# 0xC0000054/pdn-jpegxl

Hardware: AMD Instinct MI355X
Metric: megapixels/sec decode (4K lossy VarDCT) (higher is better)
Workload: dtype f32

## Files before the change

pdn_jpegxl_amd/csrc/dev_util.h:

```cpp
#pragma once
#include <stdint.h>
#include <hip/hip_fp16.h>

namespace jxlhip {

__host__ __device__ __forceinline__ int ReflectIndex(int v, int n) {
  while (v < 0 || v >= n) v = v < 0 ? -v - 1 : 2 * n - 1 - v;
  return v;
}

__host__ __device__ __forceinline__ size_t OrientedIndex(int o, int x, int y, int w, int h) {
  int ox, oy;
  switch (o) {
    case 2: ox = w - 1 - x; oy = y; break;
    case 3: ox = w - 1 - x; oy = h - 1 - y; break;
    case 4: ox = x; oy = h - 1 - y; break;
    case 5: ox = y; oy = x; break;
    case 6: ox = h - 1 - y; oy = x; break;
    case 7: ox = h - 1 - y; oy = w - 1 - x; break;
    case 8: ox = y; oy = w - 1 - x; break;
    default: ox = x; oy = y; break;
  }
  return (size_t)oy * (size_t)(o >= 5 ? h : w) + (size_t)ox;
}

__host__ __device__ __forceinline__ uint32_t NnzBucketCtx(uint32_t nzl) {
  const uint32_t b = (nzl >= 2) + (nzl >= 3) + (nzl >= 5) + (nzl >= 9) + (nzl >= 13) + (nzl >= 21) + (nzl >= 33);
  return (uint32_t)(0xCEB4987B5D3E1F00ull >> (8 * b)) & 0xFFu;
}

__host__ __device__ __forceinline__ uint32_t HfPosCtx(uint32_t ks) {
  const uint32_t a = ks - 1, b = 7 + (ks >> 1), c = 15 + (ks >> 2);
  const uint32_t bc = b < c ? b : c;
  return a < bc ? a : bc;
}

__host__ __device__ __forceinline__ uint32_t HfNnzPredict(uint32_t bx, uint32_t by, uint32_t above, uint32_t left) {
  return bx == 0 ? (by == 0 ? 32u : above) : (by == 0 ? left : (above + left + 1) >> 1);
}
__host__ __device__ __forceinline__ uint32_t HfNnzCountBucket(uint32_t predicted) {
  const uint32_t p = predicted >= 64 ? 64 : predicted;
  return p < 8 ? p : 4 + p / 2;
}

__device__ __forceinline__ uint32_t IntToOutSample(int32_t v, int bits, int out_bits) {
  const int32_t maxv = (int32_t)((1u << bits) - 1);
  if (bits == out_bits) return (uint32_t)min(maxv, max(0, v));
  float f = (float)v * (1.0f / (float)maxv);
  f *= out_bits == 16 ? 65535.0f : 255.0f;
  const float top = out_bits == 16 ? 65535.0f : 255.0f;
  if (!(f > 0.f)) return 0;
  if (f >= top) return (uint32_t)top;
  return (uint32_t)(f + 0.5f);
}

__device__ __forceinline__ float BitsToFloatSample(int32_t v, int bits) {
  if (bits == 32) return __int_as_float(v);
  return __half2float(__ushort_as_half((unsigned short)(v & 0xFFFF)));
}
__device__ __forceinline__ uint32_t FloatToOutBits(float f, int out_bits, int out_float) {
  if (out_float) return out_bits == 32 ? (uint32_t)__float_as_int(f) : (uint32_t)__half_as_ushort(__float2half_rn(f));
  const float top = out_bits == 16 ? 65535.0f : 255.0f;
  f *= top;
  if (!(f > 0.f)) return 0;
  if (f >= top) return (uint32_t)top;
  return (uint32_t)(f + 0.5f);
}
__device__ __forceinline__ uint32_t SampleToOutBits(int32_t v, int bits, int exp_bits, int out_bits, int out_float) {
  if (!out_float && !exp_bits) return IntToOutSample(v, bits, out_bits);
  const float f = exp_bits ? BitsToFloatSample(v, bits) : (float)v * (1.0f / (float)((1u << bits) - 1));
  return FloatToOutBits(f, out_bits, out_float);
}
__device__ __forceinline__ void StoreOutSample(uint8_t* base, size_t index, uint32_t raw, int out_bits) {
  if (out_bits == 8) base[index] = (uint8_t)raw;
  else if (out_bits == 16) ((uint16_t*)base)[index] = (uint16_t)raw;
  else ((uint32_t*)base)[index] = raw;
}

}
```

pdn_jpegxl_amd/csrc/entropy_kernels.hip:

```cpp
#include <hip/hip_runtime.h>
#include <cstdlib>
#include <type_traits>
#include "dev_types.h"
#include "dev_util.h"
#include "kernels.h"
#include "lds_layout.h"
#include "modular_rules.h"

namespace jxlhip {

namespace {

__device__ const uint8_t d_order_bucket[kNumStrategies] = {0, 1, 1, 1, 2, 3, 4, 4, 5, 5, 6, 6, 1, 1, 1, 1, 1, 1, 7, 8, 8, 9, 10, 10, 11, 12, 12};
__device__ const uint8_t d_log2cx[kNumStrategies] = {0, 0, 0, 0, 1, 2, 0, 1, 0, 2, 1, 2, 0, 0, 0, 0, 0, 0, 3, 2, 3, 4, 3, 4, 5, 4, 5};
__device__ const uint8_t d_log2cy[kNumStrategies] = {0, 0, 0, 0, 1, 2, 1, 0, 2, 0, 2, 1, 0, 0, 0, 0, 0, 0, 3, 3, 2, 4, 4, 3, 5, 5, 4};
__device__ const uint8_t d_nnz_ctx[64] = {0,   0,   31,  62,  62,  93,  93,  93,  93,  123, 123, 123, 123, 152, 152, 152, 152, 152, 152, 152, 152, 180,
                                          180, 180, 180, 180, 180, 180, 180, 180, 180, 180, 180, 206, 206, 206, 206, 206, 206, 206, 206, 206, 206, 206,
                                          206, 206, 206, 206, 206, 206, 206, 206, 206, 206, 206, 206, 206, 206, 206, 206, 206, 206, 206, 206};

__device__ __forceinline__ int CeilLog2D(uint32_t x) { return x <= 1 ? 0 : 32 - __clz(x - 1); }
#ifndef JXLHIP_PRIO_SERIAL
#define JXLHIP_PRIO_SERIAL 0
#endif
#if JXLHIP_PRIO_SERIAL
// ... 1090 lines not shown
    for (uint32_t i = i0; i < i1; i++) {
      const int es = s_info[i];
      s_pre[i] = base;
      base += (es >= 0 && es < kNumStrategies) ? 1u << d_log2cx[es] : 1u;
    }
    if (err & kErrBlockLayout) atomicOr(&s_flag, 1u);
  }
  __threadfence_block();
  __syncthreads();
  uint32_t num = 0;
  bool layout_bad = false;
  if (!s_flag) {
    const int words = (bw + 31) >> 5;
    for (int y = 0; y < bh; y++) {
      uint32_t pre[9];
      pre[0] = 0;
#pragma unroll
      for (int wi = 0; wi < 8; wi++) {
        uint32_t fr = 0;
        if (wi < words) {
          fr = ~s_cov[y * 8 + wi];
          const int lim = min(32, bw - wi * 32);
          if (lim < 32) fr &= (1u << lim) - 1;
        }
        pre[wi + 1] = pre[wi] + (uint32_t)__popc(fr);
      }
      const uint32_t nfree = pre[8];
      bool inrow = false, bad = false;
      if (nfree) {
        const uint32_t j = num + (uint32_t)tid;
        uint32_t off = 0;
        if (j < count) { off = s_pre[j] - s_pre[num]; inrow = off < nfree; }
        if (inrow) {
          const int es = s_info[j];
          const int lcx = d_log2cx[es], lcy = d_log2cy[es], cx = 1 << lcx, cy = 1 << lcy;
          int wi = 0;
          uint32_t before = 0;
#pragma unroll
          for (int k = 1; k < 8; k++) { const bool past = pre[k] <= off; wi += past ? 1 : 0; before = past ? pre[k] : before; }
          uint32_t word = ~s_cov[y * 8 + wi];
          const int lim = min(32, bw - wi * 32);
          if (lim < 32) word &= (1u << lim) - 1;
          uint32_t rem = off - before;
          int xb = 0;
#pragma unroll
          for (int sft = 16; sft; sft >>= 1) {
            const uint32_t c = (uint32_t)__popc((word >> xb) & ((1u << sft) - 1));
            if (rem >= c) { rem -= c; xb += sft; }
          }
          const int x = wi * 32 + xb;
          const uint32_t mask = (cx == 32 ? 0xFFFFFFFFu : ((1u << cx) - 1)) << xb;
          if (off + (uint32_t)cx > nfree || x + cx > bw || y + cy > bh || xb + cx > 32 || (y & 31) + cy > 32 || (word & mask) != mask) {
            bad = true;
          } else {
            for (int iy = 1; iy < cy; iy++)
              if (atomicOr(&s_cov[(y + iy) * 8 + wi], mask) & mask) bad = true;
            s_pos[j] = x | y << 8;
          }
        }
      }
      const int n_row = __syncthreads_count(inrow);
      if (nfree && s_pre[num + (uint32_t)n_row] - s_pre[num] != nfree) bad = true;
      if (__syncthreads_or(bad)) { layout_bad = true; break; }
      num += (uint32_t)n_row;
    }
  }
  __threadfence_block();
  __syncthreads();
  if (s_flag || layout_bad || num != count) err |= kErrBlockLayout;
  if (tid == 0) s_count = (err & kErrBlockLayout) ? 0u : num;
  __syncthreads();
  const uint32_t placed = s_count;
  for (uint32_t i = tid; i < placed; i += 256) {
    const int x = s_pos[i] & 0xFF, y = s_pos[i] >> 8;
    const int s = s_info[i], q = 1 + s_info[count + i];
    const int lcx = d_log2cx[s], lcy = d_log2cy[s], cx = 1 << lcx, cy = 1 << lcy;
    const size_t cell = (size_t)(by0 + y) * im.w8 + bx0 + x;
    for (int iy = 0; iy < cy; iy++)
      for (int ix = 0; ix < cx; ix++) {
        const size_t cc = cell + (size_t)iy * im.w8 + ix;
        im.cellinfo[cc] = (uint32_t)s | ix << 8 | iy << 13 | lcx << 18 | lcy << 21 | 1u << 31;
        im.rawq[cc] = (uint16_t)q;
      }
  }
  if (err) SetError(im, err, 2, g);
}

__global__ __launch_bounds__(64) void hf_blocklist_kernel(const DevImage* __restrict__ imgs) {
  const DevImage& im = imgs[blockIdx.y];
  const int g = blockIdx.x;
  if (g >= im.ng || im.is_modular) return;
  const int lane = threadIdx.x;
  const int gx = g % im.xg, gy = g / im.xg;
  const int bx0 = gx * kGroupBlocks, by0 = gy * kGroupBlocks;
  const int bw = min(kGroupBlocks, im.w8 - bx0), bh = min(kGroupBlocks, im.h8 - by0);
  uint32_t* list = im.blk_list + (size_t)g * 1024;
  const int n_qf = im.n_qf;
  uint32_t total = 0;
  for (int it = 0; it < 16; it++) {
    const int idx = it * 64 + lane;
    const int bx = idx & 31, by = idx >> 5;
    bool first = false;
    uint32_t info = 0;
    if (bx < bw && by < bh) {
      info = im.cellinfo[(size_t)(by0 + by) * im.w8 + bx0 + bx];
      first = (info & 0x8003FF00u) == 0x80000000u;
    }
    const uint64_t m = __ballot(first);
    if (first) {
      const uint32_t pos = total + (uint32_t)__popcll(m & (((uint64_t)1 << lane) - 1));
      const uint32_t s = info & 0xFF, lcx = (info >> 18) & 7, lcy = (info >> 21) & 7;
      const uint32_t ord = d_order_bucket[s];
      const uint32_t rq = im.rawq[(size_t)(by0 + by) * im.w8 + bx0 + bx];
      uint32_t qf_idx = 0;
      for (int i = 0; i < n_qf; i++) qf_idx += rq > im.qf_thr[i];
      uint32_t lf_idx = 0;
      if (im.num_lf_ctx > 1) {
        const size_t cell = (size_t)(by0 + by) * im.w8 + bx0 + bx;
        uint32_t ix = 0, iy = 0, ib = 0;
        for (int i = 0; i < im.n_lf_thr[0]; i++) ix += im.lfq[0][cell] > im.lf_thr[0][i];
        for (int i = 0; i < im.n_lf_thr[1]; i++) iy += im.lfq[1][cell] > im.lf_thr[1][i];
        for (int i = 0; i < im.n_lf_thr[2]; i++) ib += im.lfq[2][cell] > im.lf_thr[2][i];
        lf_idx = (ix * (uint32_t)(im.n_lf_thr[2] + 1) + ib) * (uint32_t)(im.n_lf_thr[1] + 1) + iy;
      }
      uint32_t ctxs = 0;
      for (int ci = 0; ci < 3; ci++) {
        const int c = ci == 0 ? 1 : (ci == 1 ? 0 : 2);
        const uint32_t cprime = c < 2 ? (c ^ 1) : 2;
        ctxs |= ((uint32_t)im.block_ctx_map[((cprime * kNumOrders + ord) * (n_qf + 1) + qf_idx) * im.num_lf_ctx + lf_idx] & 31u) << (5 * ci);
      }
      list[pos] = (uint32_t)bx | (uint32_t)by << 5 | lcx << 10 | lcy << 13 | ctxs << 16;
    }
    total += (uint32_t)__popcll(m);
  }
  if (lane == 0) im.blk_count[g] = total;
}

namespace {

constexpr int kHfTop = kHfRingWords / 2;
constexpr int kHfQ = kHfQueueDepth;
constexpr uint32_t kHfDqMask = 2u * kHfQ - 1;
typedef LaneBitsT<kHfRingWords, kHfRingWords / 4> HfBits;
typedef ScalarBitsT<kHfRingWords> HfScalarBits;

struct HfProfile {
#ifdef JXLHIP_PROFILE_HF
  uint64_t start = clock64(), scalar = 0, period = 0, tokens = 0, entries = 0, periods = 0, general = 0, general_n = 0;
  __device__ __forceinline__ uint64_t Now() const { return clock64(); }
  __device__ __forceinline__ void Period(uint64_t t0) { periods++; period += clock64() - t0; }
  __device__ __forceinline__ void ScalarRun(uint64_t t0, uint32_t n) { entries++; scalar += clock64() - t0; tokens += n; }
  __device__ __forceinline__ uint64_t GeneralBegin() { general_n++; return clock64(); }
  __device__ __forceinline__ void GeneralEnd(uint64_t t0) { general += clock64() - t0; }
  __device__ __forceinline__ void Print(int g, uint32_t nblk, int per_wave) const {
    if (per_wave == 1)
      printf("[hfprof] g %d total %llu scalar-loop %llu (%llu entries, %llu tokens) period %llu (%llu periods) blocks %u general %llu (%llu iterations)\n", g,
             (unsigned long long)(clock64() - start), (unsigned long long)scalar, (unsigned long long)entries, (unsigned long long)tokens,
             (unsigned long long)period, (unsigned long long)periods, nblk, (unsigned long long)general, (unsigned long long)general_n);
  }
#else
  __device__ __forceinline__ uint64_t Now() const { return 0; }
  __device__ __forceinline__ void Period(uint64_t) {}
  __device__ __forceinline__ void ScalarRun(uint64_t, uint32_t) {}
  __device__ __forceinline__ uint64_t GeneralBegin() { return 0; }
  __device__ __forceinline__ void GeneralEnd(uint64_t) {}
  __device__ __forceinline__ void Print(int, uint32_t, int) const {}
#endif
};

template <bool kLds>
struct HfLane {
  CodeTab<kLds> tab;
  typename AS<kLds>::U8 nnz_tab;
  int nslots;
  JXL_LDS uint8_t* col;
  JXL_LDS uint32_t* dq;
  const JXL_GLB uint32_t* list;
  uint32_t nblk;
  JXL_GLB uint32_t* ent;
  JXL_GLB U2* cblk;
  uint32_t ncells, w8;
  uint32_t ctx_offset, nbc;
};

struct HfQueue {
  uint32_t bi, filled, pend_n;
  uint32_t pend[kHfQ];
};

struct HfState {
  uint32_t bx, by, lcx, log2c, covered, size, ctxs, cell;
  int ci;
  uint32_t nzeros, k, prev, histo;
  bool want_nz;
  uint32_t epos;
};

template <bool kLds>
__device__ __forceinline__ void HfPeriod(const HfLane<kLds>& L, HfBits& b, HfQueue& q, HfProfile& pf) {
  const uint64_t t0 = pf.Now();
  b.TopUp();
  if (q.pend_n) {
#pragma unroll
    for (int i = 0; i < kHfQ; i++) if ((uint32_t)i < q.pend_n) L.dq[__umul24((q.filled + i) & kHfDqMask, L.nslots)] = q.pend[i];
    q.filled += q.pend_n;
    q.pend_n = 0;
  }
  if (q.filled < min(L.nblk, q.bi + kHfQ)) {
    const uint32_t lim = min(L.nblk, q.bi + kHfQ);
    uint32_t v[kHfQ];
#pragma unroll
    for (int i = 0; i < kHfQ; i++) { v[i] = 0u; if (q.filled + i < lim) v[i] = L.list[q.filled + i]; }
#pragma unroll
    for (int i = 0; i < kHfQ; i++) if (q.filled + i < lim) L.dq[__umul24((q.filled + i) & kHfDqMask, L.nslots)] = v[i];
    q.filled = lim;
  }
  {
    const uint32_t lim = min(L.nblk, q.bi + 2 * kHfQ);
    if (q.filled < lim) {
      q.pend_n = min(lim - q.filled, (uint32_t)kHfQ);
#pragma unroll
      for (int i = 0; i < kHfQ; i++) { q.pend[i] = 0u; if ((uint32_t)i < q.pend_n) q.pend[i] = L.list[q.filled + i]; }
    }
  }
  pf.Period(t0);
}

__device__ __forceinline__ int HfChannel(int ci) { return ci == 0 ? 1 : (ci == 1 ? 0 : 2); }
__device__ __forceinline__ void HfUnpackBlock(HfState& t, uint32_t d, uint32_t w8) {
  t.bx = d & 31; t.by = (d >> 5) & 31;
  t.lcx = (d >> 10) & 7;
  const uint32_t lcy = (d >> 13) & 7;
  t.ctxs = d >> 16;
  t.log2c = t.lcx + lcy; t.covered = 1u << t.log2c; t.size = t.covered << 6;
  t.cell = __umul24(t.by, w8) + t.bx;
  t.ci = 0;
}
__device__ __forceinline__ uint32_t HfNzPerCell(const HfState& t) { return (t.nzeros + t.covered - 1) >> t.log2c; }
template <bool kLds>
__device__ __forceinline__ uint32_t HfNnzCtx(const HfLane<kLds>& L, const HfState& t, int ci, uint32_t above, uint32_t left) {
  return L.ctx_offset + HfNnzCountBucket(HfNnzPredict(t.bx, t.by, above, left)) * L.nbc + ((t.ctxs >> (5 * ci)) & 31);
}
__device__ __forceinline__ uint32_t HfCoeffCtx(const HfState& t, uint32_t nz_ctx) {
  return t.histo + (nz_ctx + HfPosCtx(t.k >> t.log2c)) * 2 + t.prev;
}
template <bool kLds>
__device__ __forceinline__ bool HfTakeNnz(const HfLane<kLds>& L, HfState& t, uint32_t u) {
  t.nzeros = u;
  if (t.nzeros + t.covered > t.size) return false;
  const uint32_t fill = HfNzPerCell(t);
  const int c = HfChannel(t.ci);
  JXL_LDS uint8_t* const cc = L.col + __umul24(c * 32 + t.bx, L.nslots);
  for (uint32_t ix = 0; ix < (1u << t.lcx); ix++) cc[__umul24(ix, L.nslots)] = (uint8_t)fill;
  U2 rec;
  rec.x = t.epos; rec.y = t.nzeros;
  L.cblk[(size_t)c * L.ncells + t.cell] = rec;
  if (t.nzeros) {
    const uint32_t block_ctx = (t.ctxs >> (5 * t.ci)) & 31;
    t.histo = L.ctx_offset + L.nbc * 37 + 458 * block_ctx;
    t.prev = t.nzeros > t.size / 16 ? 0 : 1;
    t.k = t.covered;
    t.want_nz = false;
  } else {
    t.ci++;
  }
  return true;
}
template <bool kLds>
__device__ __forceinline__ bool HfTakeCoeff(const HfLane<kLds>& L, HfState& t, uint32_t u, uint32_t& err) {
  if (u) {
    const int32_t v = UnpackSigned(u);
    if (v != (int32_t)(int16_t)v) err |= kErrRange;
    L.ent[t.epos++] = t.k | (uint32_t)v << 16;
    t.prev = 1;
    if (--t.nzeros == 0) { t.want_nz = true; t.ci++; }
  } else {
    t.prev = 0;
  }
  return !(++t.k >= t.size && t.nzeros != 0);
}

template <bool kLds>
__device__ __forceinline__ void HfBatchedLoop(const HfLane<kLds>& L, HfBits& b, uint32_t& state, HfQueue& q, HfState& t, uint32_t& it, uint32_t& err,
                                              HfProfile& pf) {
  const int nslots = L.nslots;
  uint32_t nz_ctx0 = 0, nz_ctx1 = 0, nz_ctx2 = 0;
  uint32_t d_next = 0, d_after = 0;
  uint32_t up0 = 0, up1 = 0, up2 = 0, lf0 = 0, lf1 = 0, lf2 = 0;
  uint32_t pbx = 0, pcx = 0, fv0 = 0, fv1 = 0, fv2 = 0;
  while (!err) {
    if ((it & (kHfTop - 1)) == 0) HfPeriod(L, b, q, pf);
    auto colv = [&](uint32_t c, uint32_t x) { return (uint32_t)L.col[__umul24(c * 32 + x, nslots)]; };
    auto look_ahead = [&]() {
      const uint32_t x = d_next & 31, xl = x ? x - 1 : 0;
      up0 = colv(1, x); lf0 = colv(1, xl);
      up1 = colv(0, x); lf1 = colv(0, xl);
      up2 = colv(2, x); lf2 = colv(2, xl);
    };
    if (t.want_nz && t.ci >= 3) {
      if (q.bi >= L.nblk) break;
      if (q.bi == 0) {
        d_next = L.dq[0];
        d_after = L.dq[__umul24(1u & kHfDqMask, nslots)];
        look_ahead();
        pcx = 0;
      }
      HfUnpackBlock(t, d_next, L.w8);
      const uint32_t xl = t.bx ? t.bx - 1 : 0;
      const bool up_prev = t.bx - pbx < pcx, lf_prev = xl - pbx < pcx;
      nz_ctx0 = HfNnzCtx(L, t, 0, up_prev ? fv0 : up0, lf_prev ? fv0 : lf0);
      nz_ctx1 = HfNnzCtx(L, t, 1, up_prev ? fv1 : up1, lf_prev ? fv1 : lf1);
      nz_ctx2 = HfNnzCtx(L, t, 2, up_prev ? fv2 : up2, lf_prev ? fv2 : lf2);
      pbx = t.bx; pcx = 1u << t.lcx;
      q.bi++;
      d_next = d_after;
      asm volatile("" : "+v"(d_next));
      look_ahead();
      d_after = L.dq[__umul24((q.bi + 1) & kHfDqMask, nslots)];
    }
    const uint32_t nzc = t.ci == 0 ? nz_ctx0 : (t.ci == 1 ? nz_ctx1 : nz_ctx2);
    const uint32_t u = AnsGet(b, state, L.tab, t.want_nz ? nzc : HfCoeffCtx(t, NnzBucketCtx(HfNzPerCell(t))));
    it++;
    if (t.want_nz) {
      const int ci = t.ci;
      if (!HfTakeNnz(L, t, u)) { err |= kErrBitstream; break; }
      const uint32_t fill = HfNzPerCell(t);
      fv0 = ci == 0 ? fill : fv0; fv1 = ci == 1 ? fill : fv1; fv2 = ci == 2 ? fill : fv2;
    } else if (!HfTakeCoeff(L, t, u, err)) {
      err |= kErrBitstream;
      break;
    }
  }
}

template <bool kLds>
__device__ __forceinline__ void HfScalarRun(const HfLane<kLds>& L, HfBits& b, uint32_t& state, HfState& t, uint32_t& it, uint32_t& err, uint32_t cfg_uni,
                                            bool cfg_is_uni, HfProfile& pf) {
  const uint64_t t0 = pf.Now();
  uint32_t s_state = JXL_RFL(state), s_nz = JXL_RFL(t.nzeros), s_k = JXL_RFL(t.k), s_prev = JXL_RFL(t.prev), s_epos = JXL_RFL(t.epos), s_it = JXL_RFL(it);
  const uint32_t s_cov = JXL_RFL(t.covered), s_l2 = JXL_RFL(t.log2c), s_size = JXL_RFL(t.size), s_histo = JXL_RFL(t.histo);
  HfScalarBits sb;
  sb.Load(b);
  uint32_t s_rng = 0;
  const uint32_t la = JXL_RFL(L.tab.log_alpha), le = 12 - la;
  const uint32_t left = kHfTop - (s_it & (kHfTop - 1)), room = s_size > s_k ? s_size - s_k : 0u;
  const uint32_t cnt0 = min(left, room);
  uint32_t cnt = cnt0;
  uint32_t s_a = s_histo + 2 * JXL_RFL(L.nnz_tab[(s_nz + s_cov - 1) >> s_l2]);
  uint32_t s_cidx = 0xFFFFFFFFu, s_cl = 0;
  if (cnt) do {
    const uint32_t cidx = s_a + HfPosCtx(s_k >> s_l2) * 2 + s_prev;
    if (cidx != s_cidx) { s_cl = JXL_RFL(L.tab.cmap[cidx]); s_cidx = cidx; }
    const uint32_t cl = s_cl;
    const uint64_t e = L.tab.alias[(cl << la) | AnsBucket(s_state, le)];
    uint32_t c = cfg_uni;
    if (__builtin_expect(!cfg_is_uni, 0)) c = JXL_RFL(L.tab.cfg[cl]);
    const uint32_t sym = AnsStep<false>(sb, s_state, JXL_RFL((uint32_t)e), JXL_RFL((uint32_t)(e >> 32)), le);
    const uint32_t u = HybridTail(sb, c, sym);
    cnt--;
    s_prev = 0;
    if (u) {
      const int32_t v = UnpackSigned(u);
      s_rng |= (uint32_t)(v + 0x8000);
      L.ent[s_epos++] = s_k | (uint32_t)v << 16;
      s_prev = 1;
      s_k++;
      if (--s_nz == 0) break;
      s_a = s_histo + 2 * JXL_RFL(L.nnz_tab[(s_nz + s_cov - 1) >> s_l2]);
    } else {
      s_k++;
    }
  } while (cnt);
  s_it += cnt0 - cnt;
  pf.ScalarRun(t0, cnt0 - cnt);
  uint32_t s_err = s_rng > 0xFFFFu ? (uint32_t)kErrRange : 0u;
  if (s_nz != 0 && s_k >= s_size) s_err |= kErrBitstream;
  state = s_state; t.nzeros = s_nz; t.k = s_k; t.prev = s_prev; t.epos = s_epos; it = s_it;
  sb.Store(b);
  err |= s_err;
  if (s_nz == 0 && !s_err) { t.want_nz = true; t.ci++; }
}

template <bool kLds>
__device__ __forceinline__ void HfGeneralLoop(const HfLane<kLds>& L, HfBits& b, uint32_t& state, HfQueue& q, HfState& t, uint32_t& it, uint32_t& err,
                                              bool one_section, HfProfile& pf) {
  const int nslots = L.nslots;
  uint32_t cfg_uni = 0;
  bool cfg_is_uni = false;
  if (one_section) {
    cfg_uni = L.tab.cfg[0] & 0xFFF;
    cfg_is_uni = true;
    for (uint32_t i = 1; i < L.tab.dc->num_clusters; i++) cfg_is_uni &= (L.tab.cfg[i] & 0xFFF) == cfg_uni;
    cfg_uni = JXL_RFL(cfg_uni);
    cfg_is_uni = JXL_RFL(cfg_is_uni) != 0;
  }
  while (!err) {
    if ((it & (kHfTop - 1)) == 0) HfPeriod(L, b, q, pf);
    if (__all(!t.want_nz)) {
      if (one_section) {
        HfScalarRun(L, b, state, t, it, err, cfg_uni, cfg_is_uni, pf);
        continue;
      }
      for (;;) {
        const uint32_t u = AnsGet(b, state, L.tab, HfCoeffCtx(t, L.nnz_tab[HfNzPerCell(t)]));
        it++;
        const bool ok = HfTakeCoeff(L, t, u, err);
        if (!ok) err |= kErrBitstream;
        if (__any(!ok || t.want_nz) || (it & (kHfTop - 1)) == 0) break;
      }
      continue;
    }
    const uint64_t t0 = pf.GeneralBegin();
    if (t.want_nz && t.ci >= 3) {
      if (q.bi >= L.nblk) break;
      HfUnpackBlock(t, L.dq[__umul24(q.bi & kHfDqMask, nslots)], L.w8);
      q.bi++;
    }
    uint32_t ctx;
    if (t.want_nz) {
      const JXL_LDS uint8_t* const cc = L.col + __umul24(HfChannel(t.ci) * 32, nslots);
      const uint32_t xl = t.bx ? t.bx - 1 : 0;
      ctx = HfNnzCtx(L, t, t.ci, cc[__umul24(t.bx, nslots)], cc[__umul24(xl, nslots)]);
    } else {
      ctx = HfCoeffCtx(t, L.nnz_tab[HfNzPerCell(t)]);
    }
    const uint32_t u = AnsGet(b, state, L.tab, ctx);
    it++;
    if (t.want_nz) {
      if (!HfTakeNnz(L, t, u)) { err |= kErrBitstream; break; }
    } else if (!HfTakeCoeff(L, t, u, err)) {
      err |= kErrBitstream;
      break;
    }
    pf.GeneralEnd(t0);
  }
}

}

template <bool kLds>
__global__ __launch_bounds__(512) void hf_decode_kernel(const DevImage* imgs, const SectionTask* tasks, int lane_stride) {
  JXL_SERIAL_PRIO();
  extern __shared__ __align__(16) uint8_t smem[];
  const SectionTask task = tasks[blockIdx.x];
  const DevImage& im = imgs[task.image];
  const int per_wave = 64 / lane_stride;
  const int nslots = HfSlots(task.count);
  HfLane<kLds> L;
  L.nslots = nslots;
  JXL_LDS uint8_t* nzcol;
  JXL_LDS uint32_t* ring_base;
  JXL_LDS uint32_t* descq;
  {
    JXL_LDS uint8_t* lds = (JXL_LDS uint8_t*)smem;
    const HfLds at(nslots);
    ring_base = (JXL_LDS uint32_t*)(lds + at.ring);
    descq = (JXL_LDS uint32_t*)(lds + at.descq);
    nzcol = lds + at.nzcol;
    if constexpr (kLds) {
      JXL_LDS uint8_t* sn = lds + StageCode(lds, at.tables, im.acode, L.tab, threadIdx.x, blockDim.x);
      if (threadIdx.x < kNnzCtxBytes) sn[threadIdx.x] = d_nnz_ctx[threadIdx.x];
      L.nnz_tab = sn;
      __syncthreads();
    } else {
      GlobalCode(im.acode, L.tab);
      L.nnz_tab = d_nnz_ctx;
    }
  }
  if ((int)(threadIdx.x & 63) >= per_wave) return;
  const int si = (threadIdx.x >> 6) * per_wave + (threadIdx.x & 63);
  if (si >= task.count || si >= nslots) return;
  L.col = nzcol + si;
  const int g = im.hf_order[task.first + si];
  const int sec = im.single ? 0 : im.hf_sec_base + g;
  const uint64_t sec_bits = im.single ? im.hf_start_bits : im.sec_off[sec] * 8;
  HfBits b;
  b.Init(im.cs, im.cs_size, sec_bits, ring_base + si, (uint32_t)nslots);
  const uint32_t preset = b.Read(CeilLog2D((uint32_t)im.num_presets));
  L.nbc = im.num_block_ctx;
  L.ctx_offset = preset * L.nbc * 495;
  uint32_t err = preset >= (uint32_t)im.num_presets ? (uint32_t)kErrBitstream : 0u;
  if (im.lz_hf) b.SetLz(im.lz_hf + ((size_t)g << 18), 18, 0);
  uint32_t state = InitAnsState(b, L.tab);
  const int gx = g % im.xg, gy = g / im.xg;
  L.list = G(im.blk_list + (size_t)g * 1024);
// ... 669 lines not shown
```

pdn_jpegxl_amd/csrc/selftest.cc:

```cpp
#include <hip/hip_runtime.h>
#include <algorithm>
#include <cstring>
#include <stdexcept>
#include <string>
#include <vector>
#include "../../include/jxlfiletypeio.h"
#include "animation.h"
#include "dev_util.h"
#include "enc_animation.h"
#include "enc_types.h"
#include "batch_layout.h"
#include "enc_batch_layout.h"
#include "entropy_plan.h"
#include "host_parse.h"
#include "host_write.h"
#include "icc.h"
#include "modular_rules.h"

namespace jxlhip {
std::vector<EncTreeNode> MakeEncoderTree(uint32_t nlf);
extern const int32_t kWpCutsHost[kWpLeaves - 1];
std::vector<EncTreeNode> MakeLosslessSearchTree(int nch, const int32_t* pred, bool wp_ctx, int palette, uint8_t ctx[4][kWpLeaves + 1], int* palette_ctx);
void WriteLosslessSearchHeader(BitWriter& bw, int palette_colours, int palette_channels, int rct_type);
}
// ... 21 lines not shown
    std::vector<uint32_t> ctxs(n), vals(n), hist((size_t)num_ctx * kEncAlphabet, 0);
    std::vector<uint8_t> pinned(num_ctx, 0);
    if (pinned_ctx_plus1) pinned[pinned_ctx_plus1 - 1] = 1;
    for (uint32_t i = 0; i < n; i++) {
      const uint32_t c = rnd() % num_ctx;
      uint32_t v = 0;
      const uint32_t spread = 1 + c % 7;
      while ((rnd() % (spread + 1)) != 0 && v < 40) v++;
      if (rnd() % 97 == 0) v = rnd() >> (rnd() % 30);
      if (pinned[c]) v = 0;
      ctxs[i] = c; vals[i] = v;
      uint32_t tok, nb, bits;
      HybridEncode(v, &tok, &nb, &bits);
      hist[(size_t)c * kEncAlphabet + tok]++;
    }
    BitWriter bw;
    EncCode code;
    BuildAndWriteCode(hist.data(), num_ctx, max_clusters, pinned, bw, code);
    std::vector<EncToken> toks;
    for (uint32_t i = 0; i < n; i++)
      if (!pinned[ctxs[i]]) toks.push_back(EncToken{ctxs[i], vals[i]});
    WriteTokensHost(toks, code, bw);
    std::vector<uint8_t> bytes = bw.Finish();
    std::string why;
    if (!ReadBackTokens(bytes.data(), bytes.size(), num_ctx, ctxs.data(), vals.data(), n, &why)) { SetEncErr(err, why.c_str()); return 1; }
    return 0;
  } catch (const std::exception& e) {
    SetEncErr(err, e.what());
    return 2;
  }
}

extern "C" JXLFILETYPEIO_API int32_t jxlhip_selftest_tree(uint32_t nlf, ErrorInfo* err) {
  try {
    const std::vector<EncTreeNode> t = MakeEncoderTree(nlf);
    BitWriter bw;
    WriteTree(t, bw);
    std::vector<uint8_t> bytes = bw.Finish();
    std::vector<DevTreeNode> back;
    std::string why;
    if (!ReadBackTree(bytes.data(), bytes.size(), &back, &why)) { SetEncErr(err, why.c_str()); return 1; }
    if (back.size() != t.size()) { SetEncErr(err, "node count"); return 2; }
    uint32_t leaf = 0;
    for (size_t i = 0; i < t.size(); i++) {
      if (t[i].property >= 0) {
        if (back[i].property != t[i].property || back[i].splitval != t[i].splitval) { SetEncErr(err, "inner node"); return 3; }
      } else {
        if (back[i].property >= 0 || (back[i].a & 0xFF) != (uint32_t)t[i].pred || (back[i].a >> 8) != leaf || back[i].splitval != t[i].offset ||
            back[i].b != t[i].multiplier) { SetEncErr(err, "leaf"); return 4; }
        leaf++;
      }
    }
    return leaf == kNumEncLeaves ? 0 : 5;
  } catch (const std::exception& e) {
    SetEncErr(err, e.what());
    return 6;
  }
}

extern "C" JXLFILETYPEIO_API size_t jxlhip_selftest_headers(uint32_t xsize, uint32_t ysize, int32_t gray, int32_t alpha, int32_t lossless,
                                                            uint32_t epf_iters, uint32_t sec_bytes, uint8_t* dst, size_t capacity) {
  try {
    EncImageInfo ii;
    ii.xsize = xsize; ii.ysize = ysize; ii.gray = gray != 0; ii.alpha = alpha != 0; ii.xyb = !lossless;
    EncFrameInfo fi;
    fi.encoding = lossless ? 1 : 0;
    fi.gab = !lossless; fi.epf_iters = lossless ? 0 : epf_iters;
    BitWriter cs;
    WriteCodestreamHeaders(ii, cs);
    WriteFrameHeader(ii, fi, cs);
    const uint32_t ng = ((xsize + 255) / 256) * ((ysize + 255) / 256), nlf = ((xsize + 2047) / 2048) * ((ysize + 2047) / 2048);
    std::vector<uint32_t> sizes(ng == 1 ? 1 : 2 + nlf + ng, sec_bytes);
    WriteToc(sizes, cs);
    std::vector<uint8_t> bytes = cs.Finish();
    bytes.resize(bytes.size() + (size_t)sec_bytes * sizes.size(), 0);
    std::vector<uint8_t> file = WriteContainer(bytes, nullptr, 0, nullptr, 0);
    if (file.size() > capacity) return 0;
    memcpy(dst, file.data(), file.size());
    return file.size();
  } catch (...) {
    return 0;
  }
}

extern "C" JXLFILETYPEIO_API size_t jxlhip_selftest_headers_deep(uint32_t xsize, uint32_t ysize, int32_t gray, int32_t alpha, int32_t lossless,
                                                                 uint32_t bits, uint32_t exp_bits, int32_t colour, uint8_t* dst, size_t capacity) {
  try {
    EncImageInfo ii;
    ii.xsize = xsize; ii.ysize = ysize; ii.gray = gray != 0; ii.alpha = alpha != 0; ii.xyb = !lossless;
    ii.bits = bits; ii.exp_bits = exp_bits;
    switch (colour) {
      case KnownColorProfile_Srgb: case KnownColorProfile_GraySrgbTRC: break;
      case KnownColorProfile_LinearSrgb: case KnownColorProfile_LinearGray: ii.transfer = 8; break;
      case KnownColorProfile_DisplayP3: ii.primaries = 11; break;
      case KnownColorProfile_Rec709: ii.transfer = 1; break;
      case KnownColorProfile_Rec2020Linear: ii.primaries = 9; ii.transfer = 8; break;
      case KnownColorProfile_Rec2020PQ: ii.primaries = 9; ii.transfer = 16; ii.pq_intensity = true; break;
      default: return 0;
    }
    EncFrameInfo fi;
    fi.encoding = lossless ? 1 : 0;
    fi.gab = !lossless; fi.epf_iters = lossless ? 0 : 1;
    BitWriter cs;
    WriteCodestreamHeaders(ii, cs);
    WriteFrameHeader(ii, fi, cs);
    const uint32_t ng = ((xsize + 255) / 256) * ((ysize + 255) / 256), nlf = ((xsize + 2047) / 2048) * ((ysize + 2047) / 2048);
    std::vector<uint32_t> sizes(ng == 1 ? 1 : 2 + nlf + ng, 3);
    WriteToc(sizes, cs);
    std::vector<uint8_t> bytes = cs.Finish();
    bytes.resize(bytes.size() + 3 * sizes.size(), 0);
    std::vector<uint8_t> file = WriteContainer(bytes, nullptr, 0, nullptr, 0);
    if (file.size() > capacity) return 0;
    memcpy(dst, file.data(), file.size());
    return file.size();
  } catch (...) {
    return 0;
  }
}

extern "C" JXLFILETYPEIO_API size_t jxlhip_selftest_headers_icc(uint32_t xsize, uint32_t ysize, int32_t alpha, int32_t lossless, const uint8_t* icc,
                                                                size_t icc_size, uint8_t* dst, size_t capacity) {
  try {
    EncImageInfo ii;
    ii.xsize = xsize; ii.ysize = ysize; ii.gray = false; ii.alpha = alpha != 0; ii.xyb = !lossless;
    ii.icc = icc; ii.icc_size = icc_size;
    EncFrameInfo fi;
    fi.encoding = lossless ? 1 : 0;
    fi.gab = !lossless; fi.epf_iters = lossless ? 0 : 1;
    BitWriter cs;
    WriteCodestreamHeaders(ii, cs);
    WriteFrameHeader(ii, fi, cs);
    const uint32_t ng = ((xsize + 255) / 256) * ((ysize + 255) / 256), nlf = ((xsize + 2047) / 2048) * ((ysize + 2047) / 2048);
    std::vector<uint32_t> sizes(ng == 1 ? 1 : 2 + nlf + ng, 3);
    WriteToc(sizes, cs);
    std::vector<uint8_t> bytes = cs.Finish();
    bytes.resize(bytes.size() + 3 * sizes.size(), 0);
    std::vector<uint8_t> file = WriteContainer(bytes, nullptr, 0, nullptr, 0);
    if (file.size() > capacity) return 0;
    memcpy(dst, file.data(), file.size());
    return file.size();
  } catch (...) {
    return 0;
  }
}

extern "C" JXLFILETYPEIO_API int32_t jxlhip_selftest_reflect(int32_t v, int32_t n) { return ReflectIndex(v, n); }

extern "C" JXLFILETYPEIO_API uint32_t jxlhip_selftest_nnz_ctx(uint32_t nzl) { return NnzBucketCtx(nzl); }
extern "C" JXLFILETYPEIO_API uint32_t jxlhip_selftest_hf_pos_ctx(uint32_t ks) { return HfPosCtx(ks); }
extern "C" JXLFILETYPEIO_API uint32_t jxlhip_selftest_hf_nnz_predict(uint32_t bx, uint32_t by, uint32_t above, uint32_t left) {
  return HfNnzPredict(bx, by, above, left);
}
extern "C" JXLFILETYPEIO_API uint32_t jxlhip_selftest_hf_nnz_bucket(uint32_t predicted) { return HfNnzCountBucket(predicted); }

extern "C" JXLFILETYPEIO_API size_t jxlhip_selftest_write_tokens(uint32_t num_ctx, const uint32_t* ctxs, const uint32_t* values, uint32_t n,
                                                                 uint8_t* dst, size_t capacity, uint64_t* nbits) {
  try {
    std::vector<uint32_t> hist((size_t)num_ctx * kEncAlphabet, 0);
    std::vector<EncToken> toks;
    for (uint32_t i = 0; i < n; i++) {
      if (ctxs[i] >= num_ctx) return 0;
      uint32_t tok, nb, bits;
      HybridEncode(values[i], &tok, &nb, &bits);
      hist[(size_t)ctxs[i] * kEncAlphabet + tok]++;
      toks.push_back(EncToken{ctxs[i], values[i]});
    }
    BitWriter bw;
    EncCode code;
    BuildAndWriteCode(hist.data(), num_ctx, (int)num_ctx, std::vector<uint8_t>(num_ctx, 0), bw, code);
    WriteTokensHost(toks, code, bw);
    const uint64_t bit_count = bw.BitCount();
    std::vector<uint8_t> bytes = bw.Finish();
    if (bytes.size() > capacity) return 0;
    memcpy(dst, bytes.data(), bytes.size());
    *nbits = bit_count;
    return bytes.size();
  } catch (...) {
    return 0;
  }
}

extern "C" JXLFILETYPEIO_API int32_t jxlhip_selftest_lossless_tree(int32_t nch, const int32_t* pred, int32_t wp_ctx, int32_t palette, ErrorInfo* err) {
  try {
    uint8_t ctx[4][kWpLeaves + 1];
    int pal_ctx = -1;
    const std::vector<EncTreeNode> t = MakeLosslessSearchTree(nch, pred, wp_ctx != 0, palette, ctx, &pal_ctx);
    BitWriter bw;
    WriteTree(t, bw);
    std::vector<uint8_t> bytes = bw.Finish();
    std::vector<DevTreeNode> back;
    std::string why;
    if (!ReadBackTree(bytes.data(), bytes.size(), &back, &why)) { SetEncErr(err, why.c_str()); return 1; }
    if (back.size() != t.size()) { SetEncErr(err, "node count"); return 2; }
    for (size_t i = 0; i < t.size(); i++) {
      if (t[i].property >= 0 ? (back[i].property != t[i].property || back[i].splitval != t[i].splitval)
                             : (back[i].property >= 0 || (back[i].a & 0xFF) != (uint32_t)t[i].pred || back[i].b != 1 || back[i].splitval != 0)) {
        SetEncErr(err, "node differs");
        return 3;
      }
    }
    auto walk = [&](int stream, int chan, int64_t p15) {
      size_t node = 0;
      while (back[node].property >= 0) {
        const int64_t v = back[node].property == 0 ? chan : (back[node].property == 1 ? stream : p15);
        if (back[node].property != 0 && back[node].property != 1 && back[node].property != 15) throw std::runtime_error("unexpected property");
        node = v > back[node].splitval ? back[node].a : back[node].b;
      }
      return back[node].a;
    };
    for (int c = 0; c < nch; c++)
      for (int k = 0; k < kWpLeaves; k++) {
        const int64_t lo = k ? (int64_t)kWpCutsHost[k - 1] + 1 : -100000, hi = k < kWpLeaves - 1 ? (int64_t)kWpCutsHost[k] : 100000;
        for (int64_t v : {lo, hi}) {
          const int chan = palette == 1 ? c + 1 : c, stream = palette == 2 ? 21 : 0;
          const uint32_t leaf = walk(stream, chan, v);
          if ((leaf >> 8) != ctx[c][wp_ctx ? k : 0] || (leaf & 0xFF) != (uint32_t)pred[c]) { SetEncErr(err, "a walk ends in another leaf than the table says"); return 4; }
        }
      }
    if (palette) {
      const uint32_t leaf = walk(0, 0, 0);
      if ((int)(leaf >> 8) != pal_ctx || (leaf & 0xFF) != (uint32_t)pred[nch]) { SetEncErr(err, "the palette's leaf"); return 5; }
    }
    return 0;
  } catch (const std::exception& e) {
    SetEncErr(err, e.what());
    return 6;
  }
}

extern "C" JXLFILETYPEIO_API size_t jxlhip_selftest_lossless_file(uint32_t w, uint32_t h, int32_t nch, int32_t palette_colours, uint8_t* dst,
                                                                  size_t capacity) {
  try {
    if (!w || !h || w > 256 || h > 256 || nch < 1 || nch > 4 || palette_colours < 0 || palette_colours > 256) return 0;
    uint8_t ctx[4][kWpLeaves + 1];
    int pal_ctx = -1;
    std::vector<EncToken> toks;
    std::vector<EncTreeNode> tree;
    if (palette_colours) {
      const int32_t pred[2] = {5, 1};
      tree = MakeLosslessSearchTree(1, pred, false, 1, ctx, &pal_ctx);
      auto pack = [](int32_t v) { return v >= 0 ? (uint32_t)v << 1 : ((uint32_t)(-v) << 1) - 1; };
      for (int c = 0; c < nch; c++)
        for (int i = 0; i < palette_colours; i++) {
          const int32_t v = (37 * i + 91 * c) & 255, W = i ? (37 * (i - 1) + 91 * c) & 255 : (c ? (91 * (c - 1)) & 255 : 0);
          toks.push_back(EncToken{(uint32_t)pal_ctx, pack(v - W)});
        }
      auto at = [&](int x, int y) { return (int32_t)((x + 2 * y) % palette_colours); };
      for (int y = 0; y < (int)h; y++)
        for (int x = 0; x < (int)w; x++) {
          const int32_t W = x ? at(x - 1, y) : (y ? at(0, y - 1) : 0), N = x && y ? at(x, y - 1) : W, NW = x && y ? at(x - 1, y - 1) : W;
          const int32_t gr = W + N - NW, guess = std::max(std::min(W, N), std::min(std::max(W, N), gr));
          toks.push_back(EncToken{ctx[0][0], pack(at(x, y) - guess)});
        }
    } else {
      const int32_t pred[4] = {6, 6, 6, 6};
      tree = MakeLosslessSearchTree(nch, pred, true, 0, ctx, nullptr);
      for (int c = 0; c < nch; c++)
        for (uint32_t i = 0; i < w * h; i++) toks.push_back(EncToken{ctx[c][5], 0});
    }
    const size_t leaves = (tree.size() + 1) / 2;
    std::vector<uint32_t> hist(leaves * kEncAlphabet, 0);
    for (auto& t : toks) { uint32_t tok, nb, bits; HybridEncode(t.value, &tok, &nb, &bits); hist[(size_t)t.ctx * kEncAlphabet + tok]++; }
    BitWriter g;
    EncCode code;
    g.Bool(true);
    g.Bool(true);
    WriteTree(tree, g);
    BuildAndWriteCode(hist.data(), leaves, 12, {}, g, code);
    WriteLosslessSearchHeader(g, palette_colours, nch, -1);
    WriteTokensHost(toks, code, g);
    EncImageInfo ii;
    ii.xsize = w; ii.ysize = h; ii.gray = nch < 3; ii.alpha = nch == 2 || nch == 4; ii.xyb = false;
    EncFrameInfo fi;
    fi.encoding = 1; fi.group_size_shift = 1; fi.gab = false; fi.epf_iters = 0;
    BitWriter cs;
    WriteCodestreamHeaders(ii, cs);
    WriteFrameHeader(ii, fi, cs);
    std::vector<uint8_t> sec = g.Finish();
    WriteToc({(uint32_t)sec.size()}, cs);
    std::vector<uint8_t> bytes = cs.Finish();
    bytes.insert(bytes.end(), sec.begin(), sec.end());
    if (bytes.size() > capacity) return 0;
    memcpy(dst, bytes.data(), bytes.size());
    return bytes.size();
  } catch (...) {
    return 0;
  }
}

extern "C" JXLFILETYPEIO_API int32_t jxlhip_selftest_lds_layout(int32_t kind, const int64_t* in, int64_t* out) {
  int k = 0;
  auto put = [&](size_t v) { out[k++] = (int64_t)v; };
  auto shape = [&](int at) { return CodeShape{(uint32_t)in[at], (uint32_t)in[at + 1], (uint32_t)in[at + 2], in[at + 3] != 0}; };
  auto put_code = [&](const CodeLds& c) { put(c.alias); put(c.cfg); put(c.cmap); };
  if (kind == 0) {
    const CodeLds c((size_t)in[0], shape(1));
    put_code(c); put(c.end); put(CodeLdsBytes(shape(1)));
  } else if (kind == 1) {
    const ModTablesLds t((size_t)in[0], (size_t)in[1], shape(2));
    put(t.tree); put_code(CodeLds(t.code, shape(2))); put(t.end); put(ModTablesLdsBytes((size_t)in[1], shape(2)));
  } else if (kind == 2) {
    const SlotsLds l((int)in[0]);
    const ModTablesLds t(l.tables, (size_t)in[1], shape(2));
    put(0); put(t.tree); put_code(CodeLds(t.code, shape(2))); put(t.end);
    put(SlotsLdsBytes((int)in[0], (size_t)in[1], shape(2))); put(l.tables);
  } else if (kind == 3) {
// ... 563 lines not shown
```

Before: 34460.

## Make HF token loop branch-free to cut wave divergence in ANS decode

```diff
diff --git a/pdn_jpegxl_amd/csrc/dev_util.h b/pdn_jpegxl_amd/csrc/dev_util.h
--- a/pdn_jpegxl_amd/csrc/dev_util.h
+++ b/pdn_jpegxl_amd/csrc/dev_util.h
@@ -25,9 +25,11 @@
 }
 
 __host__ __device__ __forceinline__ uint32_t NnzBucketCtx(uint32_t nzl) {
-  const uint32_t b = (nzl >= 2) + (nzl >= 3) + (nzl >= 5) + (nzl >= 9) + (nzl >= 13) + (nzl >= 21) + (nzl >= 33);
-  return (uint32_t)(0xCEB4987B5D3E1F00ull >> (8 * b)) & 0xFFu;
+  const uint32_t above = (uint32_t)__builtin_popcountll(0x100101116ull >> (nzl < 63 ? nzl : 63));
+  return (uint32_t)(0x001F3E5D7B98B4CEull >> (8 * above)) & 0xFFu;
 }
+
+__host__ __device__ __forceinline__ bool HfEntryFits(int32_t v) { return v == (int32_t)(int16_t)v; }
 
 __host__ __device__ __forceinline__ uint32_t HfPosCtx(uint32_t ks) {
   const uint32_t a = ks - 1, b = 7 + (ks >> 1), c = 15 + (ks >> 2);
@@ -36,11 +38,13 @@
 }
 
 __host__ __device__ __forceinline__ uint32_t HfNnzPredict(uint32_t bx, uint32_t by, uint32_t above, uint32_t left) {
-  return bx == 0 ? (by == 0 ? 32u : above) : (by == 0 ? left : (above + left + 1) >> 1);
+  const uint32_t beside = bx == 0 ? above : left, edge = bx == 0 ? 32u : left, mean = (above + beside + 1) >> 1;
+  const uint32_t top_row = by == 0 ? ~0u : 0u;
+  return mean ^ ((mean ^ edge) & top_row);
 }
 __host__ __device__ __forceinline__ uint32_t HfNnzCountBucket(uint32_t predicted) {
-  const uint32_t p = predicted >= 64 ? 64 : predicted;
-  return p < 8 ? p : 4 + p / 2;
+  const uint32_t half = (predicted + 8) >> 1, lim = predicted < 36 ? predicted : 36;
+  return half < lim ? half : lim;
 }
 
 __device__ __forceinline__ uint32_t IntToOutSample(int32_t v, int bits, int out_bits) {
diff --git a/pdn_jpegxl_amd/csrc/entropy_kernels.hip b/pdn_jpegxl_amd/csrc/entropy_kernels.hip
--- a/pdn_jpegxl_amd/csrc/entropy_kernels.hip
+++ b/pdn_jpegxl_amd/csrc/entropy_kernels.hip
@@ -1266,13 +1266,47 @@
   __device__ __forceinline__ void ScalarRun(uint64_t t0, uint32_t n) { entries++; scalar += clock64() - t0; tokens += n; }
   __device__ __forceinline__ uint64_t GeneralBegin() { general_n++; return clock64(); }
   __device__ __forceinline__ void GeneralEnd(uint64_t t0) { general += clock64() - t0; }
+  struct ProbeBits {
+    static constexpr bool kScalar = false;
+    bool asked = false;
+    __device__ __forceinline__ uint32_t Read(int) { asked = true; return 0; }
+  };
+  uint32_t b_steps = 0, b_pops = 0, b_nnz = 0, b_coef = 0, b_tails = 0, b_renorms = 0, b_fill_cols = 0;
+  template <class Lane, class State>
+  __device__ __forceinline__ void Step(const Lane& L, const State& t, bool is_nnz, bool pop, uint32_t ctx, uint32_t state) {
+    const uint32_t cl = L.tab.cmap[ctx], le = 12 - L.tab.log_alpha;
+    ProbeBits probe;
+    uint32_t st = state;
+    const uint32_t sym = AnsStep(probe, st, L.tab.alias[(cl << L.tab.log_alpha) | AnsBucket(state, le)], le);
+    const bool tail = sym >= (1u << (L.tab.cfg[cl] & 0xF));
+    b_steps++;
+    b_pops += __any(pop) ? 1 : 0;
+    b_nnz += __any(is_nnz) ? 1 : 0;
+    b_coef += __any(!is_nnz && (tail || sym != 0)) ? 1 : 0;
+    b_tails += __any(tail) ? 1 : 0;
+    b_renorms += __any(probe.asked) ? 1 : 0;
+    for (uint32_t l = 0; l < 6; l++) b_fill_cols += __any(is_nnz && t.lcx >= l) ? (l ? 1u << (l - 1) : 1u) : 0u;
+  }
+  __device__ __forceinline__ static uint32_t WaveMax(uint32_t v) {
+    for (int m = 1; m < 64; m <<= 1) v = max(v, (uint32_t)__shfl_xor((int)v, m));
+    return v;
+  }
   __device__ __forceinline__ void Print(int g, uint32_t nblk, int per_wave) const {
-    if (per_wave == 1)
+    if (per_wave == 1) {
       printf("[hfprof] g %d total %llu scalar-loop %llu (%llu entries, %llu tokens) period %llu (%llu periods) blocks %u general %llu (%llu iterations)\n", g,
              (unsigned long long)(clock64() - start), (unsigned long long)scalar, (unsigned long long)entries, (unsigned long long)tokens,
              (unsigned long long)period, (unsigned long long)periods, nblk, (unsigned long long)general, (unsigned long long)general_n);
+      return;
+    }
+    const uint32_t steps = WaveMax(b_steps), pops = WaveMax(b_pops), nnz = WaveMax(b_nnz), coef = WaveMax(b_coef), tails = WaveMax(b_tails),
+                   renorms = WaveMax(b_renorms), fill_cols = WaveMax(b_fill_cols);
+    const uint32_t sections = (uint32_t)__popcll(__ballot(1));
+    if ((threadIdx.x & 63) == 0 && steps)
+      printf("[hfstep] workgroups %u wg %u wave %u sections %u cycles %llu steps %u pops %u nnz %u coef %u tails %u renorms %u fill_cols %u\n", gridDim.x,
+             blockIdx.x, threadIdx.x >> 6, sections, (unsigned long long)(clock64() - start), steps, pops, nnz, coef, tails, renorms, fill_cols);
   }
 #else
+  template <class Lane, class State> __device__ __forceinline__ void Step(const Lane&, const State&, bool, bool, uint32_t, uint32_t) {}
   __device__ __forceinline__ uint64_t Now() const { return 0; }
   __device__ __forceinline__ void Period(uint64_t) {}
   __device__ __forceinline__ void ScalarRun(uint64_t, uint32_t) {}
@@ -1353,26 +1387,46 @@
 __device__ __forceinline__ uint32_t HfNzPerCell(const HfState& t) { return (t.nzeros + t.covered - 1) >> t.log2c; }
 template <bool kLds>
 __device__ __forceinline__ uint32_t HfNnzCtx(const HfLane<kLds>& L, const HfState& t, int ci, uint32_t above, uint32_t left) {
-  return L.ctx_offset + HfNnzCountBucket(HfNnzPredict(t.bx, t.by, above, left)) * L.nbc + ((t.ctxs >> (5 * ci)) & 31);
+  return L.ctx_offset + __umul24(HfNnzCountBucket(HfNnzPredict(t.bx, t.by, above, left)), L.nbc) + ((t.ctxs >> (5 * ci)) & 31);
 }
 __device__ __forceinline__ uint32_t HfCoeffCtx(const HfState& t, uint32_t nz_ctx) {
   return t.histo + (nz_ctx + HfPosCtx(t.k >> t.log2c)) * 2 + t.prev;
 }
+template <bool kLds>
+__device__ __forceinline__ void HfFillColumns(const HfLane<kLds>& L, const HfState& t, int c, uint32_t fill) {
+  JXL_LDS uint8_t* const cc = L.col + __umul24(c * 32 + t.bx, L.nslots);
+  const uint32_t last = (1u << t.lcx) - 1;
+  cc[0] = (uint8_t)fill;
+  if (__any(last >= 1)) {
+    cc[__umul24(1u & last, L.nslots)] = (uint8_t)fill;
+    if (__any(last >= 2)) {
+#pragma unroll
+      for (uint32_t ix = 2; ix < 4; ix++) cc[__umul24(ix & last, L.nslots)] = (uint8_t)fill;
+      if (__any(last >= 4)) {
+#pragma unroll
+        for (uint32_t ix = 4; ix < 8; ix++) cc[__umul24(ix & last, L.nslots)] = (uint8_t)fill;
+        for (uint32_t ix = 8; __any(last >= ix); ix++) cc[__umul24(ix & last, L.nslots)] = (uint8_t)fill;
+      }
+    }
+  }
+}
+template <bool kLds>
+__device__ __forceinline__ uint32_t HfCoeffHisto(const HfLane<kLds>& L, const HfState& t) {
+  return L.ctx_offset + L.nbc * 37 + 458 * ((t.ctxs >> (5 * t.ci)) & 31);
+}
+__device__ __forceinline__ uint32_t HfFirstPrev(const HfState& t, uint32_t nzeros) { return nzeros > t.size / 16 ? 0 : 1; }
 template <bool kLds>
 __device__ __forceinline__ bool HfTakeNnz(const HfLane<kLds>& L, HfState& t, uint32_t u) {
   t.nzeros = u;
   if (t.nzeros + t.covered > t.size) return false;
-  const uint32_t fill = HfNzPerCell(t);
   const int c = HfChannel(t.ci);
-  JXL_LDS uint8_t* const cc = L.col + __umul24(c * 32 + t.bx, L.nslots);
-  for (uint32_t ix = 0; ix < (1u << t.lcx); ix++) cc[__umul24(ix, L.nslots)] = (uint8_t)fill;
+  HfFillColumns(L, t, c, HfNzPerCell(t));
   U2 rec;
   rec.x = t.epos; rec.y = t.nzeros;
   L.cblk[(size_t)c * L.ncells + t.cell] = rec;
   if (t.nzeros) {
-    const uint32_t block_ctx = (t.ctxs >> (5 * t.ci)) & 31;
-    t.histo = L.ctx_offset + L.nbc * 37 + 458 * block_ctx;
-    t.prev = t.nzeros > t.size / 16 ? 0 : 1;
+    t.histo = HfCoeffHisto(L, t);
+    t.prev = HfFirstPrev(t, t.nzeros);
     t.k = t.covered;
     t.want_nz = false;
   } else {
@@ -1384,7 +1438,7 @@
 __device__ __forceinline__ bool HfTakeCoeff(const HfLane<kLds>& L, HfState& t, uint32_t u, uint32_t& err) {
   if (u) {
     const int32_t v = UnpackSigned(u);
-    if (v != (int32_t)(int16_t)v) err |= kErrRange;
+    if (!HfEntryFits(v)) err |= kErrRange;
     L.ent[t.epos++] = t.k | (uint32_t)v << 16;
     t.prev = 1;
     if (--t.nzeros == 0) { t.want_nz = true; t.ci++; }
@@ -1392,6 +1446,33 @@
     t.prev = 0;
   }
   return !(++t.k >= t.size && t.nzeros != 0);
+}
+template <bool kLds>
+__device__ __forceinline__ bool HfTakeToken(const HfLane<kLds>& L, HfState& t, bool is_nnz, uint32_t u, uint32_t& err, uint32_t& fv0, uint32_t& fv1,
+                                            uint32_t& fv2) {
+  const bool entry = !is_nnz && u != 0;
+  const int32_t v = UnpackSigned(u);
+  err |= entry && !HfEntryFits(v) ? (uint32_t)kErrRange : 0u;
+  if (entry) L.ent[t.epos] = t.k | (uint32_t)v << 16;
+  const uint32_t owed = is_nnz ? u : t.nzeros - (entry ? 1u : 0u);
+  const bool room = u + t.covered <= t.size;
+  const bool ran_out = t.k + 1 >= t.size && owed != 0;
+  if (is_nnz && room) {
+    const uint32_t fill = (u + t.covered - 1) >> t.log2c;
+    const int c = HfChannel(t.ci);
+    HfFillColumns(L, t, c, fill);
+    fv0 = t.ci == 0 ? fill : fv0; fv1 = t.ci == 1 ? fill : fv1; fv2 = t.ci == 2 ? fill : fv2;
+    U2 rec;
+    rec.x = t.epos; rec.y = u;
+    L.cblk[(size_t)c * L.ncells + t.cell] = rec;
+    t.histo = HfCoeffHisto(L, t);
+  }
+  t.epos += entry ? 1u : 0u;
+  t.prev = is_nnz ? HfFirstPrev(t, u) : (entry ? 1u : 0u);
+  t.k = is_nnz ? t.covered : t.k + 1;
+  t.nzeros = owed;
+  t.ci += owed == 0 ? 1 : 0;
+  return is_nnz ? room : !ran_out;
 }
 
 template <bool kLds>
@@ -1402,7 +1483,8 @@
   uint32_t d_next = 0, d_after = 0;
   uint32_t up0 = 0, up1 = 0, up2 = 0, lf0 = 0, lf1 = 0, lf2 = 0;
   uint32_t pbx = 0, pcx = 0, fv0 = 0, fv1 = 0, fv2 = 0;
-  while (!err) {
+  bool done = err != 0 || L.nblk == 0;
+  while (!done) {
     if ((it & (kHfTop - 1)) == 0) HfPeriod(L, b, q, pf);
     auto colv = [&](uint32_t c, uint32_t x) { return (uint32_t)L.col[__umul24(c * 32 + x, nslots)]; };
     auto look_ahead = [&]() {
@@ -1411,8 +1493,9 @@
       up1 = colv(0, x); lf1 = colv(0, xl);
       up2 = colv(2, x); lf2 = colv(2, xl);
     };
-    if (t.want_nz && t.ci >= 3) {
-      if (q.bi >= L.nblk) break;
+    const bool is_nnz = t.nzeros == 0;
+    const bool pop = is_nnz && t.ci >= 3;
+    if (pop) {
       if (q.bi == 0) {
         d_next = L.dq[0];
         d_after = L.dq[__umul24(1u & kHfDqMask, nslots)];
@@ -1422,9 +1505,12 @@
       HfUnpackBlock(t, d_next, L.w8);
       const uint32_t xl = t.bx ? t.bx - 1 : 0;
       const bool up_prev = t.bx - pbx < pcx, lf_prev = xl - pbx < pcx;
-      nz_ctx0 = HfNnzCtx(L, t, 0, up_prev ? fv0 : up0, lf_prev ? fv0 : lf0);
-      nz_ctx1 = HfNnzCtx(L, t, 1, up_prev ? fv1 : up1, lf_prev ? fv1 : lf1);
-      nz_ctx2 = HfNnzCtx(L, t, 2, up_prev ? fv2 : up2, lf_prev ? fv2 : lf2);
+      uint32_t a0 = up_prev ? fv0 : up0, l0 = lf_prev ? fv0 : lf0, a1 = up_prev ? fv1 : up1, l1 = lf_prev ? fv1 : lf1;
+      uint32_t a2 = up_prev ? fv2 : up2, l2 = lf_prev ? fv2 : lf2;
+      asm volatile("" : "+v"(a0), "+v"(l0), "+v"(a1), "+v"(l1), "+v"(a2), "+v"(l2));
+      nz_ctx0 = HfNnzCtx(L, t, 0, a0, l0);
+      nz_ctx1 = HfNnzCtx(L, t, 1, a1, l1);
+      nz_ctx2 = HfNnzCtx(L, t, 2, a2, l2);
       pbx = t.bx; pcx = 1u << t.lcx;
       q.bi++;
       d_next = d_after;
@@ -1433,18 +1519,15 @@
       d_after = L.dq[__umul24((q.bi + 1) & kHfDqMask, nslots)];
     }
     const uint32_t nzc = t.ci == 0 ? nz_ctx0 : (t.ci == 1 ? nz_ctx1 : nz_ctx2);
-    const uint32_t u = AnsGet(b, state, L.tab, t.want_nz ? nzc : HfCoeffCtx(t, NnzBucketCtx(HfNzPerCell(t))));
+    const uint32_t ctx = is_nnz ? nzc : HfCoeffCtx(t, NnzBucketCtx(HfNzPerCell(t)));
+    pf.Step(L, t, is_nnz, pop, ctx, state);
+    const uint32_t u = AnsGet(b, state, L.tab, ctx);
     it++;
-    if (t.want_nz) {
-      const int ci = t.ci;
-      if (!HfTakeNnz(L, t, u)) { err |= kErrBitstream; break; }
-      const uint32_t fill = HfNzPerCell(t);
-      fv0 = ci == 0 ? fill : fv0; fv1 = ci == 1 ? fill : fv1; fv2 = ci == 2 ? fill : fv2;
-    } else if (!HfTakeCoeff(L, t, u, err)) {
-      err |= kErrBitstream;
-      break;
-    }
-  }
+    const bool ok = HfTakeToken(L, t, is_nnz, u, err, fv0, fv1, fv2);
+    err |= ok ? 0u : (uint32_t)kErrBitstream;
+    done = err != 0 || (t.nzeros == 0 && t.ci >= 3 && q.bi >= L.nblk);
+  }
+  t.want_nz = t.nzeros == 0;
 }
 
 template <bool kLds>
diff --git a/pdn_jpegxl_amd/csrc/selftest.cc b/pdn_jpegxl_amd/csrc/selftest.cc
--- a/pdn_jpegxl_amd/csrc/selftest.cc
+++ b/pdn_jpegxl_amd/csrc/selftest.cc
@@ -197,6 +197,7 @@
   return HfNnzPredict(bx, by, above, left);
 }
 extern "C" JXLFILETYPEIO_API uint32_t jxlhip_selftest_hf_nnz_bucket(uint32_t predicted) { return HfNnzCountBucket(predicted); }
+extern "C" JXLFILETYPEIO_API int32_t jxlhip_selftest_hf_entry_fits(uint32_t u) { return HfEntryFits(UnpackSigned(u)) ? 1 : 0; }
 
 extern "C" JXLFILETYPEIO_API size_t jxlhip_selftest_write_tokens(uint32_t num_ctx, const uint32_t* ctxs, const uint32_t* values, uint32_t n,
                                                                  uint8_t* dst, size_t capacity, uint64_t* nbits) {
```

Measured after the change: 36290, median of 6. +5.3%, better.
